# redmod-team/SympGPR

Measured on AMD Instinct MI355X. Metric: Gram-build GB/s + Cholesky fp64 TFLOP/s at N=65536 d=2; |alpha-alpha_ref|/|alpha_ref|, higher is better.
Workload: dtype f64

## Files before the change

### include/sympgpr_probe.h

```cpp
#ifndef SYMPGPR_PROBE_H
#define SYMPGPR_PROBE_H
#include <stddef.h>
#ifdef __cplusplus
extern "C" {
#endif

int sgpr_probe_mfma_f64(int waves_per_simd, int iters, double *tflops);
int sgpr_probe_hbm_write(size_t bytes, int reps, double *gbs);
int sgpr_probe_mfma_clock(int nacc, int waves_per_simd, int iters, double *out3);
int sgpr_probe_gemm(int m, int n, int k, int lower, double *out4);
int sgpr_probe_gemm_debug(int bits);
int sgpr_probe_leaf(double *out8);
int sgpr_probe_lat(double *out8);
int sgpr_probe_xcc(int nblocks, int *host_out);
int sgpr_probe_cumask(const unsigned *mask_words, int nwords, int nblocks, int *host_out);

int sgpr_probe_generated_eval(int family, int which, int m, const double *xa, const double *ya,
                              const double *xb, const double *yb, const double *l, int nl, double *out);

int sgpr_probe_queue_plan(int n, int nworkers, int *starts_out, int max_starts, unsigned *tasks_out, int max_tasks,
                          int *counts);
int sgpr_probe_queue_plan_partial(int n, int nworkers, int nq, int *starts_out, int max_starts, unsigned *tasks_out,
                                  int max_tasks, int *counts);
int sgpr_probe_queue_trace_begin(int max_tasks);
int sgpr_probe_queue_trace_end(unsigned long long *out, int max_tasks);
int sgpr_probe_queue_trace_clear(void);
int sgpr_probe_queue_postmortem(int always);
int sgpr_probe_queue_force_giveup(int on);
int sgpr_probe_tune(const char *name, double value);
int sgpr_probe_strassen_plan(int m, int n, int k, int lower, long smin, long kslab, long scratch_doubles, long long *out,
                             int max_records, int *count);
int sgpr_probe_gemm_strassen_dev(int m, int n, int k, double alpha, const double *A, size_t lda, const double *B, size_t ldb,
                                 double beta, double *C, size_t ldc, int lower, void *stream);
int sgpr_probe_gemm_nt2_dev(int m, int n, int k, double alpha, const double *A, size_t lda, const double *B, size_t ldb,
                            double beta, double *C, size_t ldc, double alpha2, double *C2, size_t ldc2, void *stream);
int sgpr_probe_strassen2_plan(int m, int n, int k, int lower, long smin, long kslab, long smin2, long kslab2, long scratch_doubles,
                              long long *out, int max_records, int *count);
int sgpr_probe_gemm_nt4_dev(int m, int n, int k, const double *A, size_t lda, const double *B, size_t ldb, double beta, int count,
                            double *const *C, const size_t *ldc, const double *alpha, void *stream);
unsigned sgpr_probe_map_calls(void);
int sgpr_probe_map_team(int ntest, int n0);

int sgpr_probe_trsm_piece(int ticket, int cap, int strips, int out[5]);
int sgpr_probe_trsm_counts(int strips, int cap, unsigned long long out[2]);

int sgpr_probe_census(int na, int threads_a, int lds_a, int spin_a, const unsigned *mask_a, int nwords_a,
                      int nb, int threads_b, int lds_b, int spin_b, const unsigned *mask_b, int nwords_b,
                      unsigned long long *host_out);

#ifdef __cplusplus
}
#endif
#endif
```

### sympgpr_amd/_lib.py

```python
import ctypes as C
import os

import numpy as np

FAMILIES = {"A": 0, "B": 1, "C": 2, "D": 3, "USER": 4}
K_KERN, K_DXDX0, K_DYDY0, K_DXDY0 = 0, 1, 2, 3
K_DLX, K_DLY = 4, 8
K_DX, K_DY, K_DX0, K_DY0, K_DXDX0DY0, K_DYDY0DY0, K_DXDY0DY0 = 16, 17, 18, 19, 20, 21, 22
G_QQ, G_PQ, G_QP, G_PP, G_ALL, G_LOWER, G_OCML, G_DLX, G_DLY = 1, 2, 4, 8, 15, 16, 32, 64, 128
FIT_LOWER_ONLY, FIT_REG, FIT_BLOCK_QQ, FIT_BLOCK_PP = 1, 4, 8, 16
MAP_WRAP_Q, MAP_WRAP_P, MAP_EXPLICIT, MAP_LOSS_NEGP = 1, 2, 4, 8
E_ARG, E_NODEVICE, E_HIP, E_NOMEM, E_STATE = -1, -2, -3, -4, -5
LOO_LPD, LOO_PRESS = 0, 1

ABI_VERSION = 5
_dp = C.POINTER(C.c_double)
_vp = C.c_void_p


class SympGPRError(RuntimeError):
    code = None
    detail = ""


# ... 118 lines not shown
PROBE_SIGNATURES = {
    "sgpr_probe_mfma_f64": (C.c_int, [C.c_int, C.c_int, _dp]),
    "sgpr_probe_mfma_clock": (C.c_int, [C.c_int, C.c_int, C.c_int, _dp]),
    "sgpr_probe_gemm": (C.c_int, [C.c_int, C.c_int, C.c_int, C.c_int, _dp]),
    "sgpr_probe_gemm_debug": (C.c_int, [C.c_int]),
    "sgpr_probe_leaf": (C.c_int, [_dp]),
    "sgpr_probe_lat": (C.c_int, [_dp]),
    "sgpr_probe_cumask": (C.c_int, [C.POINTER(C.c_uint), C.c_int, C.c_int, C.POINTER(C.c_int)]),
    "sgpr_probe_xcc": (C.c_int, [C.c_int, C.POINTER(C.c_int)]),
    "sgpr_probe_hbm_write": (C.c_int, [C.c_size_t, C.c_int, _dp]),
    "sgpr_probe_generated_eval": (C.c_int, [C.c_int, C.c_int, C.c_int, _dp, _dp, _dp, _dp, _dp, C.c_int, _dp]),
    "sgpr_probe_queue_plan": (C.c_int, [C.c_int, C.c_int, C.POINTER(C.c_int), C.c_int, C.POINTER(C.c_uint), C.c_int,
                                        C.POINTER(C.c_int)]),
    "sgpr_probe_queue_plan_partial": (C.c_int, [C.c_int, C.c_int, C.c_int, C.POINTER(C.c_int), C.c_int, C.POINTER(C.c_uint),
                                                C.c_int, C.POINTER(C.c_int)]),
    "sgpr_probe_queue_trace_begin": (C.c_int, [C.c_int]),
    "sgpr_probe_queue_trace_end": (C.c_int, [C.POINTER(C.c_ulonglong), C.c_int]),
    "sgpr_probe_queue_postmortem": (C.c_int, [C.c_int]),
    "sgpr_probe_queue_force_giveup": (C.c_int, [C.c_int]),
    "sgpr_probe_tune": (C.c_int, [C.c_char_p, C.c_double]),
    "sgpr_probe_map_calls": (C.c_uint, []),
    "sgpr_probe_map_team": (C.c_int, [C.c_int, C.c_int]),
    "sgpr_probe_trsm_piece": (C.c_int, [C.c_int, C.c_int, C.c_int, C.POINTER(C.c_int)]),
    "sgpr_probe_trsm_counts": (C.c_int, [C.c_int, C.c_int, C.POINTER(C.c_ulonglong)]),
    "sgpr_probe_queue_trace_clear": (C.c_int, []),
    "sgpr_probe_strassen_plan": (C.c_int, [C.c_int, C.c_int, C.c_int, C.c_int, C.c_long, C.c_long, C.c_long,
                                           C.POINTER(C.c_longlong), C.c_int, C.POINTER(C.c_int)]),
    "sgpr_probe_gemm_strassen_dev": (C.c_int, [C.c_int, C.c_int, C.c_int, C.c_double, C.c_void_p, C.c_size_t, C.c_void_p, C.c_size_t,
                                               C.c_double, C.c_void_p, C.c_size_t, C.c_int, C.c_void_p]),
    "sgpr_probe_gemm_nt2_dev": (C.c_int, [C.c_int, C.c_int, C.c_int, C.c_double, C.c_void_p, C.c_size_t, C.c_void_p, C.c_size_t,
                                          C.c_double, C.c_void_p, C.c_size_t, C.c_double, C.c_void_p, C.c_size_t, C.c_void_p]),
    "sgpr_probe_strassen2_plan": (C.c_int, [C.c_int, C.c_int, C.c_int, C.c_int, C.c_long, C.c_long, C.c_long, C.c_long, C.c_long,
                                            C.POINTER(C.c_longlong), C.c_int, C.POINTER(C.c_int)]),
    "sgpr_probe_gemm_nt4_dev": (C.c_int, [C.c_int, C.c_int, C.c_int, C.c_void_p, C.c_size_t, C.c_void_p, C.c_size_t, C.c_double, C.c_int,
                                          C.POINTER(C.c_void_p), C.POINTER(C.c_size_t), C.POINTER(C.c_double), C.c_void_p]),
    "sgpr_probe_census": (C.c_int, [C.c_int, C.c_int, C.c_int, C.c_int, C.POINTER(C.c_uint), C.c_int,
                                    C.c_int, C.c_int, C.c_int, C.c_int, C.POINTER(C.c_uint), C.c_int,
                                    C.POINTER(C.c_ulonglong)]),
}

_LIB = None
_PROBE = None


def load_library():
    global _LIB
    if _LIB is not None:
        return _LIB
    path = lib_path()
    if os.environ.get("SYMPGPR_NO_TORCH_PRELOAD") != "1":
        try:
            import torch
        except ImportError:
            pass
    if not os.path.exists(path):
        raise SympGPRError("%s is missing: run `python -c 'import __graft_entry__ as g; g.build()'` "
                           "(or make -C sympgpr_amd/csrc); there is no CPU fallback" % path)
    lib = C.CDLL(path)
    for name, (res, args) in SIGNATURES.items():
        fn = getattr(lib, name)
        fn.restype = res
        fn.argtypes = args
    if lib.sgpr_abi_version() != ABI_VERSION:
        raise SympGPRError("ABI version mismatch: %s is version %d, this package binds version %d -- rebuild it "
                           "(make -C sympgpr_amd/csrc)" % (path, lib.sgpr_abi_version(), ABI_VERSION))
    _LIB = lib
# ... 66 lines not shown
```

### sympgpr_amd/csrc/chol.hip

```cpp
#include <algorithm>
#include <cstdlib>
#include <mutex>
#include <vector>

#include "cholq.h"
#include "common.h"
#include "gemm_tile.h"
#include "leaf.h"

namespace sgpr {

namespace {

using namespace leaf;


__global__ __launch_bounds__(LT) void leaf_kernel(int nb, double *A, size_t lda, double *inv,
                                                  int *dinfo, int goff, int mode,
                                                  unsigned long long *stamps)
{
    __shared__ double s[LEAF_LDS];
    if (nb == LEAF) leaf_body(s, (int)LEAF, A, lda, inv, dinfo, goff, mode, stamps);
    else            leaf_body(s, nb, A, lda, inv, dinfo, goff, mode, stamps);
}
// ... 742 lines not shown
    __shared__ double s[LEAF * ILD];
    __shared__ int sh[2];
    if (threadIdx.x == 0) sh[0] = atomicAdd(q.ticket, 1);
    __syncthreads();
    const int t = sh[0];
    __syncthreads();
    const int p = t / q.G, g = t - p * q.G;
    if (p >= q.nbatch) return;
    PanelArgs a{};
    a.P = q.A + (size_t)p * q.stride_a + (size_t)q.k0 + (size_t)q.k0 * q.lda; a.lda = q.lda;
    a.W = q.W; a.R = q.R; a.G = q.G;
    a.inv = q.inv + (size_t)p * q.stride_inv + (size_t)(q.k0 / (int)LEAF) * LEAF * LEAF;
    a.dinfo = q.info + p; a.goff = q.k0;
    a.flags = q.flags + (size_t)p * PFLAG_STRIDE;
    a.below_early = 1;
    (void)panel_strip(a, g, s, sh);
}

inline int split(int n)
{
    int n1 = ((n / 2 + LEAF - 1) / LEAF) * LEAF;
    if (n1 >= n) n1 -= LEAF;
    return n1;
}

struct Ctx {
    double *inv;
    int *dinfo;
    hipStream_t st;
    int la_max = 0;
    int *flags = nullptr;
    void *qws = nullptr;
    bool strassen = false;
};

int potrf_lookahead(int n, double *A, size_t lda, const Ctx &c, int nb, int off0);
inline int la_block(int n) { return n <= 4096 ? 256 : (n <= 24576 ? 512 : (n <= 40960 ? 1024 : 2048)); }

int trsm_rec(int m, int n, const double *L, size_t ldl, double *B, size_t ldb, int off, const Ctx &c)
{
    if (n <= LEAF) {
        return gemm_nt(m, n, n, 1.0, B, ldb, c.inv + (size_t)(off / LEAF) * LEAF * LEAF, LEAF, 0.0,
                       B, ldb, 0, 0, c.st);
    }
    const int n1 = split(n), n2 = n - n1;
    int rc = trsm_rec(m, n1, L, ldl, B, ldb, off, c);
    if (rc) return rc;
    if (c.strassen) rc = gemm_nt_strassen(m, n2, n1, -1.0, B, ldb, L + n1, ldl, 1.0, B + (size_t)n1 * ldb, ldb, 0, c.st);
    else            rc = gemm_nt(m, n2, n1, -1.0, B, ldb, L + n1, ldl, 1.0, B + (size_t)n1 * ldb, ldb, 0, 0, c.st);
    if (rc) return rc;
    return trsm_rec(m, n2, L + n1 + (size_t)n1 * ldl, ldl, B + (size_t)n1 * ldb, ldb, off + n1, c);
}

int trsm_rl_rec(int m, int n, const double *L, size_t ldl, double *B, size_t ldb, int off, const Ctx &c)
{
    if (n <= LEAF)
        return gemm_nn(m, n, n, 1.0, B, ldb, c.inv + (size_t)(off / LEAF) * LEAF * LEAF, LEAF, 0.0, B, ldb, c.st);
    const int n1 = split(n), n2 = n - n1;
    int rc = trsm_rl_rec(m, n2, L + n1 + (size_t)n1 * ldl, ldl, B + (size_t)n1 * ldb, ldb, off + n1, c);
    if (rc) return rc;
    rc = gemm_nn(m, n1, n2, -1.0, B + (size_t)n1 * ldb, ldb, L + n1, ldl, 1.0, B, ldb, c.st);
    if (rc) return rc;
    return trsm_rl_rec(m, n1, L, ldl, B, ldb, off, c);
}

int potrf_rec(int n, double *A, size_t lda, int off, const Ctx &c)
{
    if (n <= LEAF) {
        hipLaunchKernelGGL(leaf_kernel, dim3(1), dim3(LT), 0, c.st, n, A, lda,
                           c.inv + (size_t)(off / LEAF) * LEAF * LEAF, c.dinfo, off, (int)LEAF_FACTOR,
                           (unsigned long long *)nullptr);
        SGPR_CHECK_LAUNCH();
        return 0;
    }
    if (n > 4 * LEAF && n <= c.la_max) return potrf_lookahead(n, A, lda, c, 0, off);
    const int n1 = split(n), n2 = n - n1;
    double *A21 = A + n1, *A22 = A + n1 + (size_t)n1 * lda;
    int rc = potrf_rec(n1, A, lda, off, c);
    if (rc) return rc;
    rc = trsm_rec(n2, n1, A, lda, A21, lda, off, c);
    if (rc) return rc;
    if (c.strassen) rc = gemm_nt_strassen(n2, n2, n1, -1.0, A21, lda, A21, lda, 1.0, A22, lda, 1, c.st);
    else            rc = gemm_nt(n2, n2, n1, -1.0, A21, lda, A21, lda, 1.0, A22, lda, 1, 0, c.st);
    if (rc) return rc;
    return potrf_rec(n2, A22, lda, off + n1, c);
}

int trsv_n_rec(int n, const double *L, size_t ldl, double *b, int off, const Ctx &c)
{
    if (n <= LEAF) {
        hipLaunchKernelGGL(leaf_matvec_kernel, dim3(1), dim3(MV_T), 0, c.st, n,
                           c.inv + (size_t)(off / LEAF) * LEAF * LEAF, b, 0);
        SGPR_CHECK_LAUNCH();
        return 0;
    }
    if (n <= TRSV_BLOCK) {
        hipLaunchKernelGGL(trsv_block_kernel, dim3(1), dim3(MV_T), 0, c.st, n, L, ldl,
                           c.inv + (size_t)(off / LEAF) * LEAF * LEAF, b, 0);
        SGPR_CHECK_LAUNCH();
        return 0;
    }
    const int n1 = split(n), n2 = n - n1;
    int rc = trsv_n_rec(n1, L, ldl, b, off, c);
    if (rc) return rc;
    rc = gemv_n_sub(n2, n1, L + n1, ldl, b, b + n1, c.st);
    if (rc) return rc;
    return trsv_n_rec(n2, L + n1 + (size_t)n1 * ldl, ldl, b + n1, off + n1, c);
}

int trsv_t_rec(int n, const double *L, size_t ldl, double *b, int off, const Ctx &c)
{
    if (n <= LEAF) {
        hipLaunchKernelGGL(leaf_matvec_kernel, dim3(1), dim3(MV_T), 0, c.st, n,
                           c.inv + (size_t)(off / LEAF) * LEAF * LEAF, b, 1);
        SGPR_CHECK_LAUNCH();
// ... 534 lines not shown
    return 0;
}

bool potrf_queue_mark_failed(hipStream_t st)
{
    const bool used = t_last_potrf_used_queue;
    if (!used) return false;
    int dev = -1;
    if ((st ? hipStreamGetDevice(st, &dev) : hipGetDevice(&dev)) != hipSuccess || dev < 0 || dev >= 64) { (void)hipGetLastError(); return false; }
    QueueDevice &qd = g_qdev[dev];
    std::lock_guard<std::mutex> lock(qd.mu);
    qd.failed = true;
    return true;
}

int potrf_trim()
{
    for (int dev = 0; dev < 64; ++dev) {
        EventPool &p = t_event_pool[dev];
        if (p.ev.empty() || p.top != 0) continue;
        for (hipEvent_t e : p.ev) (void)hipEventDestroy(e);
        p.ev.clear();
    }
    (void)hipGetLastError();
    return strassen_trim();
}

int release_device_streams(int dev)
{
    if (dev < 0 || dev >= 64) { set_error("release_device_streams: device index out of range"); return SGPR_E_ARG; }
    return release_streams(dev);
}

int potrf(int n, double *A, size_t lda, void *work, size_t lwork, int *dinfo, hipStream_t st)
{
    if (n < 0 || (n > 0 && lda < (size_t)n)) { set_error("potrf: bad n / lda"); return SGPR_E_ARG; }
    if (lwork < potrf_workspace(n)) { set_error("potrf: workspace too small"); return SGPR_E_ARG; }
    SGPR_HIP(hipMemsetAsync(dinfo, 0, sizeof(int), st));
    if (n == 0) return 0;
    int *flags = reinterpret_cast<int *>(static_cast<char *>(work) + inv_bytes(n));
    SGPR_HIP(hipMemsetAsync(flags, 0, flag_bytes(n), st));
    static const int mode = [] { const char *e = getenv("SGPR_POTRF"); return !e ? 0 : (e[0] == 'r' ? 1 : 2); }();
    static const int nb_env = [] { const char *e = getenv("SGPR_POTRF_NB"); return e ? atoi(e) : 0; }();
    static const int la_max_env = [] { const char *e = getenv("SGPR_LA_MAX"); return (int)tune("la_max", e ? atoi(e) : 57344); }();
    t_last_potrf_used_queue = false;
    Ctx c{static_cast<double *>(work), dinfo, st, mode == 1 ? 0 : la_max_env, flags};
    if (cholq::ws_bytes(n) > 0) c.qws = static_cast<char *>(work) + inv_bytes(n) + flag_bytes(n) + pub_bytes(n);
    c.strassen = true;
    if (n > c.la_max && n > LEAF) {
        const int n1 = split(n), n2 = n - n1, n11 = split(n1);
        auto need = [&](int levels) {
            return std::max(strassen_scratch_doubles(n2, n2, n1, 1, levels), strassen_scratch_doubles(n2, n1 - n11, n11, 0, levels));
        };
        strassen_reserve(need(2), need(1), st);
    }
    const bool dbg = PANEL_DBG && getenv("SGPR_PANEL_DBG") != nullptr;
    const int T = (n + LEAF - 1) / LEAF;
    if (dbg) {
        (void)hipMalloc((void **)&g_panel_dbg, sizeof(unsigned long long) * 16 * T);
        (void)hipMemset(g_panel_dbg, 0, sizeof(unsigned long long) * 16 * T);
    }
    int rc;
    if (mode == 2 || (nb_env > 0 && mode == 0 && n > 4 * LEAF && n <= c.la_max))
        rc = potrf_lookahead(n, A, lda, c, nb_env > 0 ? nb_env : 0, 0);
    else
        rc = potrf_rec(n, A, lda, 0, c);
    if (dbg) {
        (void)hipStreamSynchronize(st);
        std::vector<unsigned long long> h(16 * (size_t)T);
        (void)hipMemcpy(h.data(), g_panel_dbg, h.size() * 8, hipMemcpyDeviceToHost);
        (void)hipFree(g_panel_dbg);
        g_panel_dbg = nullptr;
        std::vector<double> d[9];
        for (int t = 1; t + 1 < T; ++t) {
            const unsigned long long *p = &h[16 * t], *q = &h[16 * (t + 1)];
            if (!p[0] || !p[5] || !q[0]) continue;
            d[0].push_back((p[1] - p[0]) * 0.01);
            d[1].push_back((p[2] - p[1]) * 0.01);
            d[2].push_back((p[3] - p[2]) * 0.01);
            d[3].push_back((p[4] - p[3]) * 0.01);
            d[4].push_back(((double)q[0] - (double)p[4]) * 0.01);
            d[5].push_back((p[5] - p[4]) * 0.01);
            d[3].back() = ((double)p[4] - (double)p[1]) * 0.01;
            d[1].back() = (p[6] - p[0]) * 0.01;
            d[2].back() = (p[7] - p[6]) * 0.01;
            d[6].push_back((p[11] - p[4]) * 0.01);
            d[7].push_back((p[12] - p[11]) * 0.01);
// ... 154 lines not shown
```

### sympgpr_amd/csrc/common.h

```cpp
#pragma once
#include <hip/hip_runtime.h>
#include <cstddef>
#include <cstdint>
#include <string>
#include <type_traits>
#include <vector>

#include "../../include/sympgpr_hip.h"

namespace sgpr {

void set_error(const std::string &msg);
double tune(const char *name, double dflt);
void tune_set(const char *name, double v);
int hip_fail(hipError_t e, const char *what, const char *file, int line);

#define SGPR_HIP(call)                                                          \
    do {                                                                        \
        hipError_t e__ = (call);                                                \
        if (e__ != hipSuccess) return ::sgpr::hip_fail(e__, #call, __FILE__, __LINE__); \
    } while (0)

#define SGPR_CHECK_LAUNCH() SGPR_HIP(hipGetLastError())

// ... 64 lines not shown
                int nhyp, const double *alpha, const double *Q0, const double *P0, double *qmap, double *pmap, int *iters,
                hipStream_t st);
int applymap_nd_tangent(int family, int d, int mode, int nm, int ntest, int n0, const double *Xtr, size_t ldxtr, const double *hyp,
                        int nhyp, const double *alpha, const double *Q0, const double *P0, double *qmap, double *pmap, int *iters,
                        double *jac, double *mono, double *lyap, hipStream_t st);
int genfun_nd(int family, int d, int m, const double *Xt, size_t ldxt, bool has_ref, int n0, const double *Xtr, size_t ldxtr,
              const double *hyp, int nhyp, const double *alpha, double *F, hipStream_t st);
int genfun_cross_nd(int family, int d, int mc, const double *Xt, size_t ldxt, const double *x0, size_t ldx0, int n0,
                    const double *Xtr, size_t ldxtr, const double *hyp, int nhyp, double *V, size_t ldv, double *prior,
                    size_t prior_stride, hipStream_t st);
bool family_is_sum(int family);

int gemm_nt(int m, int n, int k, double alpha, const double *A, size_t lda, const double *B,
            size_t ldb, double beta, double *C, size_t ldc, int lower, long diag_off,
            hipStream_t st);
int gemm_nt_bc(int m, int n, int k, double alpha, const double *A, size_t lda, const double *B,
               size_t ldb, double beta, double *C, size_t ldc, int lower, const int *bc5,
               hipStream_t st);
int gemm_nn(int m, int n, int k, double alpha, const double *A, size_t lda, const double *B, size_t ldb,
            double beta, double *C, size_t ldc, hipStream_t st);
int gemm_nt_two(int m, int n, int k, double alpha, const double *A, size_t lda, const double *B, size_t ldb, double beta,
             double *C, size_t ldc, double alpha2, double *C2, size_t ldc2, hipStream_t st);
constexpr int STRASSEN_REC = 16;
enum { PLAN_SUM = 1, PLAN_PROD = 2, PLAN_CLASSIC = 3 };
int gemm_nt_strassen(int m, int n, int k, double alpha, const double *A, size_t lda, const double *B, size_t ldb, double beta,
                     double *C, size_t ldc, int lower, hipStream_t st);
int strassen_plan(int m, int n, int k, int lower, long smin, long kslab, size_t scratch_doubles, std::vector<long long> &out);
enum { PLAN2_SUM = 4, PLAN2_PROD = 5 };
int strassen_outer_plan(int m, int n, int k, int lower, long smin, long kslab, long smin2, long kslab2, size_t scratch_doubles,
                   std::vector<long long> &out);
int gemm_nt_multi(int m, int n, int k, const double *A, size_t lda, const double *B, size_t ldb, double beta, int count,
                  double *const *C, const size_t *ldc, const double *alpha, hipStream_t st);
size_t strassen_scratch_doubles(int m, int n, int k, int lower, int levels);
void strassen_reserve(size_t both, size_t one, hipStream_t st);
int strassen_trim();
int gemm_profile_begin();
int gemm_profile_end(double *out12);
int gemm_profile_launches(double *buf, int max_records);
void gemm_set_overlap(int on);
int gemm_nt_diag(int m, int n, int k, double alpha, const double *A, size_t lda, const double *B, size_t ldb,
                 double beta, double *C, size_t ldc, int lower, unsigned long long *stamps, int dbg, hipStream_t st);

constexpr int LEAF = 128;
constexpr int POTRF_HANDOFF_TIMEOUT = -1000001;
constexpr int SOLVE_HANDOFF_TIMEOUT = -1000002;
inline int info_status(int info)
{
    if (info >= 0) return info;
    set_error(info == POTRF_HANDOFF_TIMEOUT ? "potrf: a hand-off inside the panel kernel timed out"
              : info == SOLVE_HANDOFF_TIMEOUT ? "solve: a hand-off between the strips of a triangular solve timed out" : "potrf: internal error");
    return SGPR_E_HIP;
}
size_t potrf_workspace(int n);
int potrf(int n, double *A, size_t lda, void *work, size_t lwork, int *dinfo, hipStream_t st);
size_t potrf_batch_flag_bytes(int nbatch);
int potrf_batch_max_order();
int potrf_batch(int nbatch, int npad, double *A, size_t stride_a, size_t lda, double *inv, size_t stride_inv, int *flags,
                int *info, hipStream_t st);
int potrf_batch_panel(int nbatch, int npad, int k0, int Wd, double *A, size_t stride_a, size_t lda, double *inv, size_t stride_inv,
                      int *flags, int *info, hipStream_t st);
bool potrf_queue_mark_failed(hipStream_t st);
int release_device_streams(int dev);
int trsm_rlt(int m, int n, const double *L, size_t ldl, double *B, size_t ldb, const void *work,
             hipStream_t st);
int potrs_vec(int n, const double *L, size_t ldl, void *work, double *b, hipStream_t st);
int solve_status(int n, const double *L, size_t ldl, const void *work, hipStream_t st);
// ... 97 lines not shown
```

### sympgpr_amd/csrc/gemm_f64.hip

```cpp
#include <algorithm>
#include <atomic>
#include <cstdlib>
#include <mutex>
#include <type_traits>
#include <vector>

#include "common.h"
#include "gemm_tile.h"

namespace sgpr {

namespace {

struct ProfRec { double flop; int big; int m, n, k, lower, overlap; };
struct Prof {
    std::mutex mu;
    std::atomic<bool> on{false};
    std::vector<hipEvent_t> pool;
    std::vector<ProfRec> recs;
    long dropped = 0;
};
constexpr int PROF_POOL = 8192;
Prof g_prof;
thread_local int t_overlap = 0;
// ... 389 lines not shown
        put(out, {PLAN_CLASSIC, 1, r0, 0, r0, 0, n, n, k, r0, r0});
        return;
    }
    plan_syrk(h, k, r0, c, out);
    plan_gemm(h, h, k, r0 + h, r0, r0 + h, r0, c, out);
    plan_syrk(h, k, r0 + h, c, out);
}
size_t plan_need(const std::vector<long long> &plan)
{
    size_t need[2] = {0, 0};
    for (size_t i = 0; i + STRASSEN_REC <= plan.size(); i += STRASSEN_REC)
        if (plan[i] == PLAN_SUM) need[plan[i + 1]] = std::max(need[plan[i + 1]], (size_t)plan[i + 2] * (size_t)plan[i + 3]);
    return need[0] + need[1];
}

int strassen_levels()
{
    static const int lv = [] { const char *e = getenv("SGPR_GEMM_STRASSEN"); return !e ? 2 : (e[0] == '0' ? 0 : (e[0] == '1' ? 1 : 2)); }();
    return lv;
}
bool strassen_on() { return strassen_levels() > 0; }
PlanCfg default_cfg()
{
    static const long smin = std::max(128L, (long)tune("gemm_strassen_min", 8192));
    static const long kslab = std::max(32L, (long)tune("gemm_strassen_kslab", 16384));
    return PlanCfg{smin, kslab, ~(size_t)0};
}

struct Plan2Cfg {
    PlanCfg in;
    long smin2;
    long kslab2;
    size_t scratch;
};
Plan2Cfg default_cfg2()
{
    static const long smin2 = std::max(256L, (long)tune("gemm_strassen2_min", 16384));
    static const long kslab2 = std::max(64L, (long)tune("gemm_strassen2_kslab", 32768));
    return Plan2Cfg{default_cfg(), smin2, kslab2, ~(size_t)0};
}
bool outer_noscratch()
{
    static const bool forced_fail = tune("gemm_strassen2_noscratch", 0) != 0;
    return forced_fail;
}
bool qualifies2(long m, long n, long k, const Plan2Cfg &c)
{
    if (m <= 0 || n <= 0 || m % 1024 != 0 || n % 512 != 0) return false;
    if (m / 2 < c.smin2 || n / 2 < c.smin2) return false;
    if (c.kslab2 < 64 || c.kslab2 % 64 != 0 || k < c.kslab2) return false;
    const size_t pair = (size_t)(m / 2 + n / 2) * (size_t)(c.kslab2 / 2);
    if (pair > c.scratch) return false;
    PlanCfg ci = c.in;
    ci.scratch = c.scratch - pair;
    return qualifies(m / 2, n / 2, c.kslab2 / 2, ci);
}
PlanCfg inner_of(const Plan2Cfg &c)
{
    PlanCfg ci = c.in;
    ci.scratch = c.scratch;
    return ci;
}
void plan2_gemm(long m, long n, long k, long ar, long br, long cr, long cc, const Plan2Cfg &c, std::vector<long long> &out)
{
    if (!qualifies2(m, n, k, c)) { plan_gemm(m, n, k, ar, br, cr, cc, inner_of(c), out); return; }
    long k0 = 0;
    for (; k0 + c.kslab2 <= k; k0 += c.kslab2) seven(PLAN2_SUM, PLAN2_PROD, m / 2, n / 2, c.kslab2 / 2, k0, ar, br, cr, cc, out);
    if (k0 == k) return;
    size_t i = out.size();
    plan_gemm(m, n, k - k0, ar, br, cr, cc, inner_of(c), out);
    for (; i + STRASSEN_REC <= out.size(); i += STRASSEN_REC) {
        long long *r = &out[i];
        if (r[0] == PLAN_SUM) { r[5] += k0; r[7] += k0; }
        else if (r[0] == PLAN_PROD) { if (!r[1]) r[3] += k0; if (!r[4]) r[6] += k0; }
        else { r[3] += k0; r[5] += k0; }
    }
}
void plan2_syrk(long n, long k, long r0, const Plan2Cfg &c, std::vector<long long> &out)
{
    const long h = n / 2;
    if (n % 2 != 0 || !qualifies2(h, h, k, c)) { plan_syrk(n, k, r0, inner_of(c), out); return; }
    plan2_syrk(h, k, r0, c, out);
    plan2_gemm(h, h, k, r0 + h, r0, r0 + h, r0, c, out);
    plan2_syrk(h, k, r0 + h, c, out);
}
void inner_plan(const long long *r, const PlanCfg &ci, std::vector<long long> &out)
{
    out.clear();
    plan_gemm(r[7], r[8], r[9], 0, 0, 0, 0, ci, out);
}
struct Need2 { size_t v[4] = {0, 0, 0, 0}; size_t inner() const { return v[0] + v[1]; } size_t total() const { return v[0] + v[1] + v[2] + v[3]; } };
Need2 plan2_need(const std::vector<long long> &plan, const Plan2Cfg &c)
{
    Need2 nd;
    std::vector<long long> in;
    auto sums = [&](const long long *r, int base) {
        size_t &v = nd.v[base + r[1]];
        v = std::max(v, (size_t)r[2] * (size_t)r[3]);
    };
    PlanCfg ci = c.in;
    ci.scratch = ~(size_t)0;
    for (size_t i = 0; i + STRASSEN_REC <= plan.size(); i += STRASSEN_REC) {
        const long long *r = &plan[i];
        if (r[0] == PLAN_SUM) sums(r, 0);
        else if (r[0] == PLAN2_SUM) sums(r, 2);
        else if (r[0] == PLAN2_PROD) {
            inner_plan(r, ci, in);
            for (size_t j = 0; j + STRASSEN_REC <= in.size(); j += STRASSEN_REC)
                if (in[j] == PLAN_SUM) sums(&in[j], 0);
        }
    }
    return nd;
}

struct Scratch {
    std::mutex mu;
    double *p = nullptr;
    size_t cap = 0, failed = 0;
    hipEvent_t ev = nullptr;
    hipStream_t last = nullptr;
    bool used = false;
};
Scratch g_scratch[64];

bool scratch_ensure(Scratch &s, size_t need)
{
    static const bool forced_fail = tune("gemm_strassen_noscratch", 0) != 0;
    if (forced_fail) return false;
    if (s.cap >= need) return true;
    if (s.failed && need >= s.failed) return false;
    if (s.p) { (void)hipFree(s.p); s.p = nullptr; s.cap = 0; s.used = false; }
    if (hipMalloc((void **)&s.p, need * sizeof(double)) != hipSuccess) {
        (void)hipGetLastError();
// ... 45 lines not shown
                if (r[15]) add(C + r[13] + (size_t)r[14] * ldc, ldc, alpha * (double)r[15]);
                add(C2 + r[10] + (size_t)r[11] * ldc2, ldc2, alpha2 * (double)r[12]);
                if (r[15]) add(C2 + r[13] + (size_t)r[14] * ldc2, ldc2, alpha2 * (double)r[15]);
                if (cnt == 2) rc = gemm_nt_two(m, n, k, as[0], Ap, la, Bp, lb, 1.0, cs[0], ls[0], as[1], cs[1], ls[1], st);
                else          rc = gemm_nt_multi(m, n, k, Ap, la, Bp, lb, 1.0, cnt, cs, ls, as, st);
            } else if (r[15]) {
                rc = gemm_nt_two(m, n, k, alpha * (double)r[12], Ap, la, Bp, lb, 1.0, C1, ldc,
                                 alpha * (double)r[15], C + r[13] + (size_t)r[14] * ldc, ldc, st);
            } else {
                rc = gemm_nt(m, n, k, alpha * (double)r[12], Ap, la, Bp, lb, 1.0, C1, ldc, 0, 0, st);
            }
        } else if (r[0] == PLAN_CLASSIC) {
            const double *Ap = A + r[2] + (size_t)r[3] * lda, *Bp = B + r[4] + (size_t)r[5] * ldb;
            if (C2) rc = gemm_nt_two((int)r[6], (int)r[7], (int)r[8], alpha, Ap, lda, Bp, ldb, beta, C + r[9] + (size_t)r[10] * ldc, ldc,
                                     alpha2, C2 + r[9] + (size_t)r[10] * ldc2, ldc2, st);
            else    rc = gemm_nt((int)r[6], (int)r[7], (int)r[8], alpha, Ap, lda, Bp, ldb, beta, C + r[9] + (size_t)r[10] * ldc, ldc, (int)r[1], 0, st);
        } else {
            set_error("run_plan: unknown record");
            rc = SGPR_E_ARG;
        }
        if (rc) return rc;
    }
    return 0;
}
int run_plan(const std::vector<long long> &plan, double alpha, const double *A, size_t lda, const double *B, size_t ldb,
             double beta, double *C, size_t ldc, double *SA, double *SB, hipStream_t st)
{
    return run_plan(plan.data(), plan.size() / STRASSEN_REC, alpha, A, lda, B, ldb, beta, C, ldc, 0.0, nullptr, 0, SA, SB, st);
}
int run_plan2(const std::vector<long long> &plan, const Plan2Cfg &c, const Need2 &nd, double alpha, const double *A, size_t lda,
              const double *B, size_t ldb, double beta, double *C, size_t ldc, double *S, hipStream_t st)
{
    double *const SA = S, *const SB = S + nd.v[0], *const OA = SB + nd.v[1], *const OB = OA + nd.v[2];
    PlanCfg ci = c.in;
    ci.scratch = nd.inner();
    std::vector<long long> in;
    for (size_t i = 0; i + STRASSEN_REC <= plan.size(); i += STRASSEN_REC) {
        const long long *r = &plan[i];
        int rc = 0;
        if (r[0] == PLAN2_SUM) {
            const double *P = r[1] ? B : A;
            const size_t ld = r[1] ? ldb : lda;
            rc = block_sum((int)r[2], (int)r[3], P + r[4] + (size_t)r[5] * ld, ld, P + r[6] + (size_t)r[7] * ld, ld, (double)r[8],
                           r[1] ? OB : OA, st);
        } else if (r[0] == PLAN2_PROD) {
            const double *X = r[1] ? OA : A + r[2] + (size_t)r[3] * lda;
            const double *Y = r[4] ? OB : B + r[5] + (size_t)r[6] * ldb;
            inner_plan(r, ci, in);
            rc = run_plan(in.data(), in.size() / STRASSEN_REC, alpha * (double)r[12], X, r[1] ? (size_t)r[7] : lda, Y, r[4] ? (size_t)r[8] : ldb,
                          1.0, C + r[10] + (size_t)r[11] * ldc, ldc, alpha * (double)r[15], r[15] ? C + r[13] + (size_t)r[14] * ldc : nullptr, ldc,
                          SA, SB, st);
        } else {
            rc = run_plan(r, 1, alpha, A, lda, B, ldb, beta, C, ldc, 0.0, nullptr, 0, SA, SB, st);
        }
        if (rc) return rc;
    }
    return 0;
}
}

int strassen_plan(int m, int n, int k, int lower, long smin, long kslab, size_t scratch_doubles, std::vector<long long> &out)
{
    if (m < 0 || n < 0 || k < 0 || (lower && m != n)) { set_error("strassen_plan: bad extents"); return SGPR_E_ARG; }
    PlanCfg c = default_cfg();
    if (smin >= 0) c.smin = std::max(128L, smin);
    if (kslab >= 0) c.kslab = std::max(32L, kslab);
    c.scratch = scratch_doubles;
    out.clear();
    if (lower) plan_syrk(n, k, 0, c, out);
    else       plan_gemm(m, n, k, 0, 0, 0, 0, c, out);
    return 0;
}

namespace {
Plan2Cfg cfg2_of(long smin, long kslab, long smin2, long kslab2, size_t scratch_doubles)
{
    Plan2Cfg c = default_cfg2();
    if (smin >= 0) c.in.smin = std::max(128L, smin);
    if (kslab >= 0) c.in.kslab = std::max(32L, kslab);
    if (smin2 >= 0) c.smin2 = std::max(256L, smin2);
    if (kslab2 >= 0) c.kslab2 = std::max(64L, kslab2);
    c.scratch = scratch_doubles;
    return c;
}
}

int strassen_outer_plan(int m, int n, int k, int lower, long smin, long kslab, long smin2, long kslab2, size_t scratch_doubles,
                   std::vector<long long> &out)
{
    if (m < 0 || n < 0 || k < 0 || (lower && m != n)) { set_error("strassen_outer_plan: bad extents"); return SGPR_E_ARG; }
    const Plan2Cfg c = cfg2_of(smin, kslab, smin2, kslab2, scratch_doubles);
    out.clear();
    if (lower) plan2_syrk(n, k, 0, c, out);
    else       plan2_gemm(m, n, k, 0, 0, 0, 0, c, out);
    return 0;
}

size_t strassen_scratch_doubles(int m, int n, int k, int lower, int levels)
{
    std::vector<long long> plan;
    if (!strassen_on()) return 0;
    if (levels >= 2 && strassen_levels() >= 2) {
        if (strassen_outer_plan(m, n, k, lower, -1, -1, -1, -1, ~(size_t)0, plan)) return 0;
        return plan2_need(plan, default_cfg2()).total();
    }
    if (strassen_plan(m, n, k, lower, -1, -1, ~(size_t)0, plan)) return 0;
    return plan_need(plan);
}

void strassen_reserve(size_t both, size_t one, hipStream_t st)
{
    const int dev = device_of(st);
    if (dev < 0 || !strassen_on()) return;
    Scratch &s = g_scratch[dev];
    std::lock_guard<std::mutex> lock(s.mu);
    if (both > one && !outer_noscratch() && scratch_ensure(s, both)) return;
    if (one) (void)scratch_ensure(s, one);
}

int strassen_trim()
{
    for (Scratch &s : g_scratch) {
        std::lock_guard<std::mutex> lock(s.mu);
        if (s.p) (void)hipFree(s.p);
        if (s.ev) (void)hipEventDestroy(s.ev);
        s.p = nullptr; s.ev = nullptr; s.cap = 0; s.failed = 0; s.used = false; s.last = nullptr;
    }
    (void)hipGetLastError();
    return 0;
}

int gemm_nt_strassen(int m, int n, int k, double alpha, const double *A, size_t lda, const double *B, size_t ldb, double beta,
                     double *C, size_t ldc, int lower, hipStream_t st)
{
    const bool aligned = ((((uintptr_t)A | (uintptr_t)B) & 15) == 0) && (((lda | ldb) & 1) == 0);
    if (std::min(m, n) / 2 < default_cfg().smin || !strassen_on() || !aligned || beta != 1.0 || (lower && m != n))
        return gemm_nt(m, n, k, alpha, A, lda, B, ldb, beta, C, ldc, lower, 0, st);
    std::vector<long long> plan;
    int rc = 0;
    const int dev = device_of(st);
    auto enqueue = [&](Scratch &s, auto &&run) {
        if (!s.ev) SGPR_HIP(hipEventCreateWithFlags(&s.ev, hipEventDisableTiming));
        if (s.used && s.last != st) SGPR_HIP(hipStreamWaitEvent(st, s.ev, 0));
        const int r = run();
        SGPR_HIP(hipEventRecord(s.ev, st));
        s.last = st;
        s.used = true;
        return r;
    };
    const Plan2Cfg c2 = default_cfg2();
    if (strassen_levels() >= 2 && dev >= 0 && !outer_noscratch() && std::min(lower ? m / 2 : m, lower ? n / 2 : n) / 2 >= c2.smin2) {
        if ((rc = strassen_outer_plan(m, n, k, lower, -1, -1, -1, -1, ~(size_t)0, plan))) return rc;
        const Need2 nd = plan2_need(plan, c2);
        if (nd.v[2] + nd.v[3]) {
            Scratch &s = g_scratch[dev];
            std::lock_guard<std::mutex> lock(s.mu);
            if (scratch_ensure(s, nd.total()))
                return enqueue(s, [&] { return run_plan2(plan, c2, nd, alpha, A, lda, B, ldb, beta, C, ldc, s.p, st); });
        }
    }
    rc = strassen_plan(m, n, k, lower, -1, -1, ~(size_t)0, plan);
    if (rc) return rc;
    const size_t need = plan_need(plan);
    if (!need) return run_plan(plan, alpha, A, lda, B, ldb, beta, C, ldc, nullptr, nullptr, st);
    if (dev < 0) return gemm_nt(m, n, k, alpha, A, lda, B, ldb, beta, C, ldc, lower, 0, st);
    Scratch &s = g_scratch[dev];
    std::lock_guard<std::mutex> lock(s.mu);
    if (!scratch_ensure(s, need)) {
        if ((rc = strassen_plan(m, n, k, lower, -1, -1, s.cap, plan))) return rc;
        if (!plan_need(plan)) return run_plan(plan, alpha, A, lda, B, ldb, beta, C, ldc, nullptr, nullptr, st);
    }
    size_t na = 0;
    for (size_t i = 0; i + STRASSEN_REC <= plan.size(); i += STRASSEN_REC)
        if (plan[i] == PLAN_SUM && plan[i + 1] == 0) na = std::max(na, (size_t)plan[i + 2] * (size_t)plan[i + 3]);
    return enqueue(s, [&] { return run_plan(plan, alpha, A, lda, B, ldb, beta, C, ldc, s.p, s.p + na, st); });
}

}
```

### sympgpr_amd/csrc/probe.hip

```cpp
#include <algorithm>
#include <cstdlib>
#include <vector>

#include "cholq.h"
#include "common.h"
#include "../../include/sympgpr_probe.h"
#include "generated/pair_generated.h"

namespace sgpr {
namespace {
typedef double double4_t __attribute__((ext_vector_type(4)));
typedef double double2_t __attribute__((ext_vector_type(2)));

template <int NACC>
__global__ __launch_bounds__(256) void mfma_clock_kernel(int iters, double *out, unsigned long long *stamps)
{
    double4_t acc[NACC];
    const double a = 1.0 + threadIdx.x * 1e-9, b = 1.0 - threadIdx.x * 1e-9;
#pragma unroll
    for (int i = 0; i < NACC; ++i) acc[i] = double4_t{0.0, 0.0, 0.0, 0.0};
    const unsigned long long t0 = __builtin_amdgcn_s_memtime(), r0 = __builtin_amdgcn_s_memrealtime();
    for (int it = 0; it < iters; ++it) {
#pragma unroll
        for (int i = 0; i < NACC; ++i)
// ... 478 lines not shown

extern "C" int sgpr_probe_strassen_plan(int m, int n, int k, int lower, long smin, long kslab, long scratch_doubles, long long *out,
                                        int max_records, int *count)
{
    if (!count || scratch_doubles < 0) { set_error("probe_strassen_plan: bad arguments"); return SGPR_E_ARG; }
    std::vector<long long> plan;
    const int rc = strassen_plan(m, n, k, lower, smin, kslab, (size_t)scratch_doubles, plan);
    if (rc) return rc;
    *count = (int)(plan.size() / STRASSEN_REC);
    for (size_t i = 0; out && i < plan.size() && (int)(i / STRASSEN_REC) < max_records; ++i) out[i] = plan[i];
    return 0;
}
extern "C" int sgpr_probe_gemm_strassen_dev(int m, int n, int k, double alpha, const double *A, size_t lda, const double *B, size_t ldb,
                                            double beta, double *C, size_t ldc, int lower, void *stream)
{
    return gemm_nt_strassen(m, n, k, alpha, A, lda, B, ldb, beta, C, ldc, lower, static_cast<hipStream_t>(stream));
}
extern "C" int sgpr_probe_gemm_nt2_dev(int m, int n, int k, double alpha, const double *A, size_t lda, const double *B, size_t ldb,
                                       double beta, double *C, size_t ldc, double alpha2, double *C2, size_t ldc2, void *stream)
{
    return gemm_nt_two(m, n, k, alpha, A, lda, B, ldb, beta, C, ldc, alpha2, C2, ldc2, static_cast<hipStream_t>(stream));
}
extern "C" int sgpr_probe_strassen2_plan(int m, int n, int k, int lower, long smin, long kslab, long smin2, long kslab2,
                                         long scratch_doubles, long long *out, int max_records, int *count)
{
    if (!count || scratch_doubles < 0) { set_error("probe_strassen2_plan: bad arguments"); return SGPR_E_ARG; }
    std::vector<long long> plan;
    const int rc = strassen_outer_plan(m, n, k, lower, smin, kslab, smin2, kslab2, (size_t)scratch_doubles, plan);
    if (rc) return rc;
    *count = (int)(plan.size() / STRASSEN_REC);
    for (size_t i = 0; out && i < plan.size() && (int)(i / STRASSEN_REC) < max_records; ++i) out[i] = plan[i];
    return 0;
}
extern "C" int sgpr_probe_gemm_nt4_dev(int m, int n, int k, const double *A, size_t lda, const double *B, size_t ldb, double beta,
                                       int count, double *const *C, const size_t *ldc, const double *alpha, void *stream)
{
    return gemm_nt_multi(m, n, k, A, lda, B, ldb, beta, count, C, ldc, alpha, static_cast<hipStream_t>(stream));
}
extern "C" unsigned sgpr_probe_map_calls(void) { return applymap_last_calls(); }
extern "C" int sgpr_probe_map_team(int ntest, int n0) { return applymap_team(ntest, n0); }
extern "C" int sgpr_probe_trsm_piece(int ticket, int cap, int strips, int out[5]) { if (ticket < 0 || cap < 1 || strips < 0 || !out) return SGPR_E_ARG; trsm_piece_of(ticket, cap, strips, out); return 0; }
extern "C" int sgpr_probe_trsm_counts(int strips, int cap, unsigned long long out[2])
{
    if (strips < 0 || cap < 1 || !out) return SGPR_E_ARG;
    size_t c[2];
    trsm_piece_counts(strips, cap, c);
    out[0] = c[0]; out[1] = c[1];
    return 0;
}

namespace sgpr { namespace {
__global__ void census_kernel(unsigned long long *out, int spin_us)
{
    extern __shared__ double dyn[];
    const unsigned long long t0 = __builtin_amdgcn_s_memrealtime();
    if (threadIdx.x == 0) {
        dyn[0] = 1.0;
        out[4 * blockIdx.x + 0] = (unsigned long long)__builtin_amdgcn_s_getreg(20 | (0 << 6) | (3 << 11));
        out[4 * blockIdx.x + 1] = (unsigned long long)__builtin_amdgcn_s_getreg(4 | (0 << 6) | (31 << 11));
        out[4 * blockIdx.x + 2] = t0;
    }
    while (__builtin_amdgcn_s_memrealtime() - t0 < (unsigned long long)spin_us * 100ull) __builtin_amdgcn_s_sleep(32);
    if (threadIdx.x == 0) out[4 * blockIdx.x + 3] = __builtin_amdgcn_s_memrealtime();
}
} }
extern "C" int sgpr_probe_census(int na, int threads_a, int lds_a, int spin_a, const unsigned *mask_a, int nwords_a,
// ... 31 lines not shown
```

Before: 79.26.

## Use lower Strassen thresholds and short k-slabs in recursive Cholesky updates

Adds a per-call Strassen configuration so the recursive potrf/trsm updates can use smaller Strassen cut-offs (separate for GEMM and SYRK), a separate inner-level threshold under the two-level scheme, and a shorter outer k-slab when k is moderate. Scratch reservation now walks the whole recursion tree to size the buffer for the largest update, not just the top two calls. The aim is to apply Strassen's reduced flop count to more of the mid-sized trailing updates. In exchange it adds extra additions and memory traffic on smaller blocks and may cost fp64 accuracy.

```diff
diff --git a/include/sympgpr_probe.h b/include/sympgpr_probe.h
--- a/include/sympgpr_probe.h
+++ b/include/sympgpr_probe.h
@@ -38,6 +38,11 @@
                               long long *out, int max_records, int *count);
 int sgpr_probe_gemm_nt4_dev(int m, int n, int k, const double *A, size_t lda, const double *B, size_t ldb, double beta, int count,
                             double *const *C, const size_t *ldc, const double *alpha, void *stream);
+int sgpr_probe_strassen_rec_plan(int m, int n, int k, int lower, long scratch_doubles, long cfg_out[5], long long *out,
+                                 int max_records, int *count);
+int sgpr_probe_strassen_rec_scratch(int n, unsigned long long out[2]);
+int sgpr_probe_gemm_strassen_rec_dev(int m, int n, int k, double alpha, const double *A, size_t lda, const double *B, size_t ldb,
+                                     double beta, double *C, size_t ldc, int lower, void *stream);
 unsigned sgpr_probe_map_calls(void);
 int sgpr_probe_map_team(int ntest, int n0);
 
diff --git a/sympgpr_amd/_lib.py b/sympgpr_amd/_lib.py
--- a/sympgpr_amd/_lib.py
+++ b/sympgpr_amd/_lib.py
@@ -174,6 +174,11 @@
                                           C.c_double, C.c_void_p, C.c_size_t, C.c_double, C.c_void_p, C.c_size_t, C.c_void_p]),
     "sgpr_probe_strassen2_plan": (C.c_int, [C.c_int, C.c_int, C.c_int, C.c_int, C.c_long, C.c_long, C.c_long, C.c_long, C.c_long,
                                             C.POINTER(C.c_longlong), C.c_int, C.POINTER(C.c_int)]),
+    "sgpr_probe_strassen_rec_plan": (C.c_int, [C.c_int, C.c_int, C.c_int, C.c_int, C.c_long, C.POINTER(C.c_long),
+                                               C.POINTER(C.c_longlong), C.c_int, C.POINTER(C.c_int)]),
+    "sgpr_probe_strassen_rec_scratch": (C.c_int, [C.c_int, C.POINTER(C.c_ulonglong)]),
+    "sgpr_probe_gemm_strassen_rec_dev": (C.c_int, [C.c_int, C.c_int, C.c_int, C.c_double, C.c_void_p, C.c_size_t, C.c_void_p, C.c_size_t,
+                                                   C.c_double, C.c_void_p, C.c_size_t, C.c_int, C.c_void_p]),
     "sgpr_probe_gemm_nt4_dev": (C.c_int, [C.c_int, C.c_int, C.c_int, C.c_void_p, C.c_size_t, C.c_void_p, C.c_size_t, C.c_double, C.c_int,
                                           C.POINTER(C.c_void_p), C.POINTER(C.c_size_t), C.POINTER(C.c_double), C.c_void_p]),
     "sgpr_probe_census": (C.c_int, [C.c_int, C.c_int, C.c_int, C.c_int, C.POINTER(C.c_uint), C.c_int,
diff --git a/sympgpr_amd/csrc/chol.hip b/sympgpr_amd/csrc/chol.hip
--- a/sympgpr_amd/csrc/chol.hip
+++ b/sympgpr_amd/csrc/chol.hip
@@ -798,6 +798,7 @@
     int *flags = nullptr;
     void *qws = nullptr;
     bool strassen = false;
+    StrassenRec rec;
 };
 
 int potrf_lookahead(int n, double *A, size_t lda, const Ctx &c, int nb, int off0);
@@ -812,7 +813,7 @@
     const int n1 = split(n), n2 = n - n1;
     int rc = trsm_rec(m, n1, L, ldl, B, ldb, off, c);
     if (rc) return rc;
-    if (c.strassen) rc = gemm_nt_strassen(m, n2, n1, -1.0, B, ldb, L + n1, ldl, 1.0, B + (size_t)n1 * ldb, ldb, 0, c.st);
+    if (c.strassen) rc = gemm_nt_strassen_cfg(m, n2, n1, -1.0, B, ldb, L + n1, ldl, 1.0, B + (size_t)n1 * ldb, ldb, 0, strassen_rec_cfg(c.rec, n1, 0), c.st);
     else            rc = gemm_nt(m, n2, n1, -1.0, B, ldb, L + n1, ldl, 1.0, B + (size_t)n1 * ldb, ldb, 0, 0, c.st);
     if (rc) return rc;
     return trsm_rec(m, n2, L + n1 + (size_t)n1 * ldl, ldl, B + (size_t)n1 * ldb, ldb, off + n1, c);
@@ -846,7 +847,7 @@
     if (rc) return rc;
     rc = trsm_rec(n2, n1, A, lda, A21, lda, off, c);
     if (rc) return rc;
-    if (c.strassen) rc = gemm_nt_strassen(n2, n2, n1, -1.0, A21, lda, A21, lda, 1.0, A22, lda, 1, c.st);
+    if (c.strassen) rc = gemm_nt_strassen_cfg(n2, n2, n1, -1.0, A21, lda, A21, lda, 1.0, A22, lda, 1, strassen_rec_cfg(c.rec, n1, 1), c.st);
     else            rc = gemm_nt(n2, n2, n1, -1.0, A21, lda, A21, lda, 1.0, A22, lda, 1, 0, c.st);
     if (rc) return rc;
     return potrf_rec(n2, A22, lda, off + n1, c);
@@ -1447,6 +1448,40 @@
     return release_streams(dev);
 }
 
+namespace {
+int la_max_value()
+{
+    static const int v = [] { const char *e = getenv("SGPR_LA_MAX"); return (int)tune("la_max", e ? atoi(e) : 57344); }();
+    return v;
+}
+void need_trsm(int m, int n, const StrassenRec &v, int levels, size_t &need)
+{
+    if (n <= LEAF || std::min(m, n) < 256) return;
+    const int n1 = split(n), n2 = n - n1;
+    need_trsm(m, n1, v, levels, need);
+    need = std::max(need, strassen_scratch_doubles_cfg(m, n2, n1, 0, levels, strassen_rec_cfg(v, n1, 0)));
+    need_trsm(m, n2, v, levels, need);
+}
+void need_potrf(int n, int la_max, const StrassenRec &v, int levels, size_t &need)
+{
+    if (n <= LEAF || (n > 4 * LEAF && n <= la_max)) return;
+    const int n1 = split(n), n2 = n - n1;
+    need_potrf(n1, la_max, v, levels, need);
+    need_trsm(n2, n1, v, levels, need);
+    need = std::max(need, strassen_scratch_doubles_cfg(n2, n2, n1, 1, levels, strassen_rec_cfg(v, n1, 1)));
+    need_potrf(n2, la_max, v, levels, need);
+}
+}
+
+void potrf_strassen_need(int n, size_t out[2])
+{
+    static const bool rec_mode = [] { const char *e = getenv("SGPR_POTRF"); return e && e[0] == 'r'; }();
+    const StrassenRec v = strassen_rec_values();
+    out[0] = out[1] = 0;
+    need_potrf(n, rec_mode ? 0 : la_max_value(), v, 2, out[0]);
+    need_potrf(n, rec_mode ? 0 : la_max_value(), v, 1, out[1]);
+}
+
 int potrf(int n, double *A, size_t lda, void *work, size_t lwork, int *dinfo, hipStream_t st)
 {
     if (n < 0 || (n > 0 && lda < (size_t)n)) { set_error("potrf: bad n / lda"); return SGPR_E_ARG; }
@@ -1457,17 +1492,16 @@
     SGPR_HIP(hipMemsetAsync(flags, 0, flag_bytes(n), st));
     static const int mode = [] { const char *e = getenv("SGPR_POTRF"); return !e ? 0 : (e[0] == 'r' ? 1 : 2); }();
     static const int nb_env = [] { const char *e = getenv("SGPR_POTRF_NB"); return e ? atoi(e) : 0; }();
-    static const int la_max_env = [] { const char *e = getenv("SGPR_LA_MAX"); return (int)tune("la_max", e ? atoi(e) : 57344); }();
+    const int la_max_env = la_max_value();
     t_last_potrf_used_queue = false;
     Ctx c{static_cast<double *>(work), dinfo, st, mode == 1 ? 0 : la_max_env, flags};
     if (cholq::ws_bytes(n) > 0) c.qws = static_cast<char *>(work) + inv_bytes(n) + flag_bytes(n) + pub_bytes(n);
     c.strassen = true;
+    c.rec = strassen_rec_values();
     if (n > c.la_max && n > LEAF) {
-        const int n1 = split(n), n2 = n - n1, n11 = split(n1);
-        auto need = [&](int levels) {
-            return std::max(strassen_scratch_doubles(n2, n2, n1, 1, levels), strassen_scratch_doubles(n2, n1 - n11, n11, 0, levels));
-        };
-        strassen_reserve(need(2), need(1), st);
+        size_t need[2];
+        potrf_strassen_need(n, need);
+        strassen_reserve(need[0], need[1], st);
     }
     const bool dbg = PANEL_DBG && getenv("SGPR_PANEL_DBG") != nullptr;
     const int T = (n + LEAF - 1) / LEAF;
diff --git a/sympgpr_amd/csrc/common.h b/sympgpr_amd/csrc/common.h
--- a/sympgpr_amd/csrc/common.h
+++ b/sympgpr_amd/csrc/common.h
@@ -120,6 +120,17 @@
 int gemm_nt_multi(int m, int n, int k, const double *A, size_t lda, const double *B, size_t ldb, double beta, int count,
                   double *const *C, const size_t *ldc, const double *alpha, hipStream_t st);
 size_t strassen_scratch_doubles(int m, int n, int k, int lower, int levels);
+struct StrassenCfg { long smin = -1, kslab = -1, smin2 = -1, kslab2 = -1, smin_under = -1; };
+int gemm_nt_strassen_cfg(int m, int n, int k, double alpha, const double *A, size_t lda, const double *B, size_t ldb, double beta,
+                         double *C, size_t ldc, int lower, const StrassenCfg &cfg, hipStream_t st);
+size_t strassen_scratch_doubles_cfg(int m, int n, int k, int lower, int levels, const StrassenCfg &cfg);
+struct StrassenRec { bool on = false; long smin_gemm = 0, smin_syrk = 0, smin2_gemm = 0, smin2_syrk = 0, kslab = 0, kslab2 = 0, kslab2_short = 0; };
+StrassenRec strassen_rec_values();
+StrassenCfg strassen_rec_cfg(const StrassenRec &v, int k, int lower);
+int strassen_rec_plan(int m, int n, int k, int lower, long cfg_out[5], size_t scratch_doubles, std::vector<long long> &out);
+int gemm_nt_strassen_rec(int m, int n, int k, double alpha, const double *A, size_t lda, const double *B, size_t ldb, double beta,
+                         double *C, size_t ldc, int lower, hipStream_t st);
+void potrf_strassen_need(int n, size_t out[2]);
 void strassen_reserve(size_t both, size_t one, hipStream_t st);
 int strassen_trim();
 int gemm_profile_begin();
diff --git a/sympgpr_amd/csrc/gemm_f64.hip b/sympgpr_amd/csrc/gemm_f64.hip
--- a/sympgpr_amd/csrc/gemm_f64.hip
+++ b/sympgpr_amd/csrc/gemm_f64.hip
@@ -445,7 +445,15 @@
     long smin2;
     long kslab2;
     size_t scratch;
+    long smin_under = -1;
 };
+PlanCfg under_of(const Plan2Cfg &c)
+{
+    PlanCfg ci = c.in;
+    if (c.smin_under >= 0) ci.smin = c.smin_under;
+    return ci;
+}
+constexpr long REC_SMIN_GEMM = 4096, REC_SMIN_SYRK = 8192, REC_SMIN2_GEMM = 8192, REC_SMIN2_SYRK = 8192, REC_KSLAB2_SHORT = 16384;
 Plan2Cfg default_cfg2()
 {
     static const long smin2 = std::max(256L, (long)tune("gemm_strassen2_min", 16384));
@@ -464,7 +472,7 @@
     if (c.kslab2 < 64 || c.kslab2 % 64 != 0 || k < c.kslab2) return false;
     const size_t pair = (size_t)(m / 2 + n / 2) * (size_t)(c.kslab2 / 2);
     if (pair > c.scratch) return false;
-    PlanCfg ci = c.in;
+    PlanCfg ci = under_of(c);
     ci.scratch = c.scratch - pair;
     return qualifies(m / 2, n / 2, c.kslab2 / 2, ci);
 }
@@ -511,7 +519,7 @@
         size_t &v = nd.v[base + r[1]];
         v = std::max(v, (size_t)r[2] * (size_t)r[3]);
     };
-    PlanCfg ci = c.in;
+    PlanCfg ci = under_of(c);
     ci.scratch = ~(size_t)0;
     for (size_t i = 0; i + STRASSEN_REC <= plan.size(); i += STRASSEN_REC) {
         const long long *r = &plan[i];
@@ -623,7 +631,7 @@
               const double *B, size_t ldb, double beta, double *C, size_t ldc, double *S, hipStream_t st)
 {
     double *const SA = S, *const SB = S + nd.v[0], *const OA = SB + nd.v[1], *const OB = OA + nd.v[2];
-    PlanCfg ci = c.in;
+    PlanCfg ci = under_of(c);
     ci.scratch = nd.inner();
     std::vector<long long> in;
     for (size_t i = 0; i + STRASSEN_REC <= plan.size(); i += STRASSEN_REC) {
@@ -674,28 +682,77 @@
     c.scratch = scratch_doubles;
     return c;
 }
-}
-
-int strassen_outer_plan(int m, int n, int k, int lower, long smin, long kslab, long smin2, long kslab2, size_t scratch_doubles,
-                   std::vector<long long> &out)
-{
-    if (m < 0 || n < 0 || k < 0 || (lower && m != n)) { set_error("strassen_outer_plan: bad extents"); return SGPR_E_ARG; }
-    const Plan2Cfg c = cfg2_of(smin, kslab, smin2, kslab2, scratch_doubles);
+Plan2Cfg cfg2_of(const StrassenCfg &cfg, size_t scratch_doubles)
+{
+    Plan2Cfg c = cfg2_of(cfg.smin, cfg.kslab, cfg.smin2, cfg.kslab2, scratch_doubles);
+    if (cfg.smin_under >= 0) c.smin_under = std::max(128L, cfg.smin_under);
+    return c;
+}
+void outer_plan_of(int m, int n, int k, int lower, const Plan2Cfg &c, std::vector<long long> &out)
+{
     out.clear();
     if (lower) plan2_syrk(n, k, 0, c, out);
     else       plan2_gemm(m, n, k, 0, 0, 0, 0, c, out);
+}
+}
+
+int strassen_outer_plan(int m, int n, int k, int lower, long smin, long kslab, long smin2, long kslab2, size_t scratch_doubles,
+                   std::vector<long long> &out)
+{
+    if (m < 0 || n < 0 || k < 0 || (lower && m != n)) { set_error("strassen_outer_plan: bad extents"); return SGPR_E_ARG; }
+    outer_plan_of(m, n, k, lower, cfg2_of(smin, kslab, smin2, kslab2, scratch_doubles), out);
+    return 0;
+}
+
+StrassenRec strassen_rec_values()
+{
+    StrassenRec v;
+    v.on = getenv("SGPR_GEMM_STRASSEN") == nullptr;
+    const Plan2Cfg lib = default_cfg2();
+    v.smin_gemm = std::max(128L, (long)tune("rec_strassen_min_gemm", std::min(REC_SMIN_GEMM, lib.in.smin)));
+    v.smin_syrk = std::max(128L, (long)tune("rec_strassen_min_syrk", std::min(REC_SMIN_SYRK, lib.in.smin)));
+    v.smin2_gemm = std::max(256L, (long)tune("rec_strassen2_min_gemm", std::min(REC_SMIN2_GEMM, lib.smin2)));
+    v.smin2_syrk = std::max(256L, (long)tune("rec_strassen2_min_syrk", std::min(REC_SMIN2_SYRK, lib.smin2)));
+    v.kslab = std::max(32L, (long)tune("rec_strassen_kslab", lib.in.kslab));
+    v.kslab2 = std::max(64L, (long)tune("rec_strassen2_kslab", lib.kslab2));
+    v.kslab2_short = (long)tune("rec_strassen2_kslab_short", REC_KSLAB2_SHORT);
+    if (v.kslab2_short < 64 || v.kslab2_short % 64 != 0 || v.kslab2_short >= v.kslab2) v.kslab2_short = 0;
+    return v;
+}
+StrassenCfg strassen_rec_cfg(const StrassenRec &v, int k, int lower)
+{
+    StrassenCfg c;
+    if (!v.on) return c;
+    c.smin = lower ? v.smin_syrk : v.smin_gemm;
+    c.smin2 = lower ? v.smin2_syrk : v.smin2_gemm;
+    c.smin_under = std::min(c.smin, c.smin2 / 2);
+    c.kslab = v.kslab;
+    c.kslab2 = (k < v.kslab2 && v.kslab2_short > 0 && k >= v.kslab2_short) ? v.kslab2_short : v.kslab2;
+    return c;
+}
+int strassen_rec_plan(int m, int n, int k, int lower, long cfg_out[5], size_t scratch_doubles, std::vector<long long> &out)
+{
+    if (m < 0 || n < 0 || k < 0 || (lower && m != n)) { set_error("strassen_rec_plan: bad extents"); return SGPR_E_ARG; }
+    const Plan2Cfg c = cfg2_of(strassen_rec_cfg(strassen_rec_values(), k, lower), scratch_doubles);
+    if (cfg_out) { cfg_out[0] = c.in.smin; cfg_out[1] = c.in.kslab; cfg_out[2] = c.smin2; cfg_out[3] = c.kslab2; cfg_out[4] = under_of(c).smin; }
+    outer_plan_of(m, n, k, lower, c, out);
     return 0;
 }
 
 size_t strassen_scratch_doubles(int m, int n, int k, int lower, int levels)
 {
+    return strassen_scratch_doubles_cfg(m, n, k, lower, levels, StrassenCfg{});
+}
+size_t strassen_scratch_doubles_cfg(int m, int n, int k, int lower, int levels, const StrassenCfg &cfg)
+{
     std::vector<long long> plan;
-    if (!strassen_on()) return 0;
+    if (!strassen_on() || m < 0 || n < 0 || k < 0 || (lower && m != n)) return 0;
+    const Plan2Cfg c2 = cfg2_of(cfg, ~(size_t)0);
     if (levels >= 2 && strassen_levels() >= 2) {
-        if (strassen_outer_plan(m, n, k, lower, -1, -1, -1, -1, ~(size_t)0, plan)) return 0;
-        return plan2_need(plan, default_cfg2()).total();
-    }
-    if (strassen_plan(m, n, k, lower, -1, -1, ~(size_t)0, plan)) return 0;
+        outer_plan_of(m, n, k, lower, c2, plan);
+        return plan2_need(plan, c2).total();
+    }
+    if (strassen_plan(m, n, k, lower, c2.in.smin, c2.in.kslab, ~(size_t)0, plan)) return 0;
     return plan_need(plan);
 }
 
@@ -724,8 +781,19 @@
 int gemm_nt_strassen(int m, int n, int k, double alpha, const double *A, size_t lda, const double *B, size_t ldb, double beta,
                      double *C, size_t ldc, int lower, hipStream_t st)
 {
+    return gemm_nt_strassen_cfg(m, n, k, alpha, A, lda, B, ldb, beta, C, ldc, lower, StrassenCfg{}, st);
+}
+int gemm_nt_strassen_rec(int m, int n, int k, double alpha, const double *A, size_t lda, const double *B, size_t ldb, double beta,
+                         double *C, size_t ldc, int lower, hipStream_t st)
+{
+    return gemm_nt_strassen_cfg(m, n, k, alpha, A, lda, B, ldb, beta, C, ldc, lower, strassen_rec_cfg(strassen_rec_values(), k, lower), st);
+}
+int gemm_nt_strassen_cfg(int m, int n, int k, double alpha, const double *A, size_t lda, const double *B, size_t ldb, double beta,
+                         double *C, size_t ldc, int lower, const StrassenCfg &cfg, hipStream_t st)
+{
+    const Plan2Cfg c2 = cfg2_of(cfg, ~(size_t)0);
     const bool aligned = ((((uintptr_t)A | (uintptr_t)B) & 15) == 0) && (((lda | ldb) & 1) == 0);
-    if (std::min(m, n) / 2 < default_cfg().smin || !strassen_on() || !aligned || beta != 1.0 || (lower && m != n))
+    if (std::min(m, n) / 2 < std::min(c2.in.smin, under_of(c2).smin) || !strassen_on() || !aligned || beta != 1.0 || (lower && m != n))
         return gemm_nt(m, n, k, alpha, A, lda, B, ldb, beta, C, ldc, lower, 0, st);
     std::vector<long long> plan;
     int rc = 0;
@@ -739,9 +807,8 @@
         s.used = true;
         return r;
     };
-    const Plan2Cfg c2 = default_cfg2();
     if (strassen_levels() >= 2 && dev >= 0 && !outer_noscratch() && std::min(lower ? m / 2 : m, lower ? n / 2 : n) / 2 >= c2.smin2) {
-        if ((rc = strassen_outer_plan(m, n, k, lower, -1, -1, -1, -1, ~(size_t)0, plan))) return rc;
+        outer_plan_of(m, n, k, lower, c2, plan);
         const Need2 nd = plan2_need(plan, c2);
         if (nd.v[2] + nd.v[3]) {
             Scratch &s = g_scratch[dev];
@@ -750,7 +817,7 @@
                 return enqueue(s, [&] { return run_plan2(plan, c2, nd, alpha, A, lda, B, ldb, beta, C, ldc, s.p, st); });
         }
     }
-    rc = strassen_plan(m, n, k, lower, -1, -1, ~(size_t)0, plan);
+    rc = strassen_plan(m, n, k, lower, c2.in.smin, c2.in.kslab, ~(size_t)0, plan);
     if (rc) return rc;
     const size_t need = plan_need(plan);
     if (!need) return run_plan(plan, alpha, A, lda, B, ldb, beta, C, ldc, nullptr, nullptr, st);
@@ -758,7 +825,7 @@
     Scratch &s = g_scratch[dev];
     std::lock_guard<std::mutex> lock(s.mu);
     if (!scratch_ensure(s, need)) {
-        if ((rc = strassen_plan(m, n, k, lower, -1, -1, s.cap, plan))) return rc;
+        if ((rc = strassen_plan(m, n, k, lower, c2.in.smin, c2.in.kslab, s.cap, plan))) return rc;
         if (!plan_need(plan)) return run_plan(plan, alpha, A, lda, B, ldb, beta, C, ldc, nullptr, nullptr, st);
     }
     size_t na = 0;
diff --git a/sympgpr_amd/csrc/probe.hip b/sympgpr_amd/csrc/probe.hip
--- a/sympgpr_amd/csrc/probe.hip
+++ b/sympgpr_amd/csrc/probe.hip
@@ -534,6 +534,30 @@
     for (size_t i = 0; out && i < plan.size() && (int)(i / STRASSEN_REC) < max_records; ++i) out[i] = plan[i];
     return 0;
 }
+extern "C" int sgpr_probe_strassen_rec_plan(int m, int n, int k, int lower, long scratch_doubles, long cfg_out[5], long long *out,
+                                            int max_records, int *count)
+{
+    if (!count || scratch_doubles < 0) { set_error("probe_strassen_rec_plan: bad arguments"); return SGPR_E_ARG; }
+    std::vector<long long> plan;
+    const int rc = strassen_rec_plan(m, n, k, lower, cfg_out, (size_t)scratch_doubles, plan);
+    if (rc) return rc;
+    *count = (int)(plan.size() / STRASSEN_REC);
+    for (size_t i = 0; out && i < plan.size() && (int)(i / STRASSEN_REC) < max_records; ++i) out[i] = plan[i];
+    return 0;
+}
+extern "C" int sgpr_probe_strassen_rec_scratch(int n, unsigned long long out[2])
+{
+    if (n < 0 || !out) { set_error("probe_strassen_rec_scratch: bad arguments"); return SGPR_E_ARG; }
+    size_t need[2];
+    potrf_strassen_need(n, need);
+    out[0] = need[0]; out[1] = need[1];
+    return 0;
+}
+extern "C" int sgpr_probe_gemm_strassen_rec_dev(int m, int n, int k, double alpha, const double *A, size_t lda, const double *B, size_t ldb,
+                                                double beta, double *C, size_t ldc, int lower, void *stream)
+{
+    return gemm_nt_strassen_rec(m, n, k, alpha, A, lda, B, ldb, beta, C, ldc, lower, static_cast<hipStream_t>(stream));
+}
 extern "C" int sgpr_probe_gemm_nt4_dev(int m, int n, int k, const double *A, size_t lda, const double *B, size_t ldb, double beta,
                                        int count, double *const *C, const size_t *ldc, const double *alpha, void *stream)
 {
```

After: 80.98, median of 6. 1.02x the previous value.
